# astrodeepnet/debvader

Measured on AMD Instinct MI355X. Metric: galaxy stamps/sec (train fwd+bwd+Adam) 59x59x6, higher is better.
Workload: dtype f32; 1 GPU; BASELINE configs[1]: 6-band 59x59 stamps, batch=256 per GPU, latent_dim=32, filters [32,64,128,256], fp32, stage-1 VAE train step; global_batch=256, per_gpu_batch=256, parallelism=dp1

## Files before the change

### debvader_amd/csrc/common.h

```cpp
#pragma once
#include <hip/hip_runtime.h>
#include <stdint.h>
#include <stddef.h>
#include <memory>
#include <utility>
#include <vector>

namespace dv {

enum : int {
  OK = 0,
  E_INVALID = -1,
  E_HIP = -2,
  E_NOMEM = -3,
  E_RCCL = -4,
  E_STATE = -5,
  E_NODEVICE = -6,
};

void set_error(const char* fmt, ...);
int hip_fail(hipError_t e, const char* what, const char* file, int line);

#define DV_HIP(call)                                                     \
  do {                                                                   \
// ... 65 lines not shown
__device__ __forceinline__ void dv_philox4x32_10(unsigned c0, unsigned c1, unsigned c2, unsigned c3, unsigned k0,
                                                 unsigned k1, unsigned out[4]) {
#pragma unroll
  for (int r = 0; r < 10; ++r) {
    unsigned long long p0 = 0xD2511F53ull * c0, p1 = 0xCD9E8D57ull * c2;
    unsigned n0 = (unsigned)(p1 >> 32) ^ c1 ^ k0, n1 = (unsigned)p1;
    unsigned n2 = (unsigned)(p0 >> 32) ^ c3 ^ k1, n3 = (unsigned)p0;
    c0 = n0; c1 = n1; c2 = n2; c3 = n3;
    k0 += 0x9E3779B9u;
    k1 += 0xBB67AE85u;
  }
  out[0] = c0; out[1] = c1; out[2] = c2; out[3] = c3;
}
__device__ __forceinline__ float dv_philox_normal(unsigned row, unsigned col, unsigned stream, unsigned long long seed) {
  unsigned r[4];
  dv_philox4x32_10(row, col >> 2, stream, 0u, (unsigned)seed, (unsigned)(seed >> 32), r);
  const int a = col & 3;
  const float u1 = ((float)r[a & ~1] + 1.0f) * 2.3283064365386963e-10f;
  const float u2 = ((float)r[(a & ~1) + 1] + 1.0f) * 2.3283064365386963e-10f;
  const float rad = sqrtf(-2.0f * logf(fminf(u1, 1.0f)));
  float sn, cs;
  sincosf(6.283185307179586f * u2, &sn, &cs);
  return (a & 1) ? rad * sn : rad * cs;
}
#endif

#define DV_MAX_TAPS 25
struct TapTab {
  int n;
  unsigned t[DV_MAX_TAPS];
};

struct GConvParams {
  const float* X;
  const float* W;
  float* U;
  float* A;
  const float* bias;
  const float* alpha;
  int NB, Hin, Win, Cin;
  int Hout, Wout, Cout;
  int Hc, Wc;
  int sin, sout, ph, pw;
  int ntaps;
  TapTab xt;
  int M, K;
// ... 227 lines not shown
struct DetectDevSrc {
  const double* fields_dev;
  int nb, band;
  const int32_t* which_h;
};
int scene_detect_dev(const DetectDevSrc& src, int M, int H, int W, double thresh, double cont, int minarea, int nthresh,
                     int back_size, int back_filter, const double* kernel_h, int kh, int kw, int64_t workspace_bytes,
                     int64_t cap, int64_t* n_out, int64_t* offsets_h, double* globalrms_h, int32_t* field_h,
                     int32_t* parent_h, int32_t* npix_h, double* peak_h, double* flux_h, double* x_h, double* y_h,
                     hipStream_t s);

struct GStripParams {
  const float* X;
  const float* W;
  float* U;
  float* A;
  const float* bias;
  const float* alpha;
  const float* zero;
  int NB, H, Wd, Cin, Cout;
  unsigned long long tapcode, wtcode;
  int epi;
  int R, patch_floats, strips_per_stamp, nstrips, strips_per_wg;
};
int launch_gconv_strip(GStripParams p, bool nmajor, hipStream_t s);
int launch_gconv_strip8(GStripParams p, hipStream_t s);

struct WinoParams {
  const float* X;
  const float* Ut;
  float* U;
  float* A;
  const float* bias;
  const float* alpha;
  const float* zero;
  int NB, H, Cin, Cout;
  int epi;
  int nbh, nct, NC, groups, items, items_per_wg;
};
struct WinoWDesc {
  const float* W;
  float* Ut;
  int Cin, Cout, nmajor;
  int wtmap[9];
};
struct WinoWgradParams {
  const float* X;
  const float* Y;
// ... 210 lines not shown
```

### debvader_amd/csrc/engine.hip

```cpp
#include <rccl/rccl.h>
#include <math.h>
#include <stdarg.h>
#include <stdio.h>
#include <stdlib.h>
#include <string.h>
#include <unistd.h>

#include <algorithm>
#include <string>
#include <thread>
#include <map>
#include <memory>
#include <mutex>
#include <optional>
#include <set>
#include <vector>
#ifdef DV_DEBUG_EXPORTS
#include <functional>
#endif

#include "../../include/debvader_hip.h"
#ifdef DV_DEBUG_EXPORTS
#include "../../include/debvader_hip_debug.h"
#endif
// ... 334 lines not shown
  hipEvent_t ev_red = nullptr;
  hipStream_t lane_stream[3] = {nullptr, nullptr, nullptr};
  hipEvent_t ev_lane[3] = {nullptr, nullptr, nullptr};
  hipEvent_t ev_ready = nullptr, ev_join = nullptr, ev_buf[3] = {nullptr, nullptr, nullptr};
  hipEvent_t ev_dec = nullptr, ev_enc = nullptr, ev_comm = nullptr, ev_small = nullptr, ev_small2 = nullptr;
  hipEvent_t ev_mid = nullptr;
  hipEvent_t ev_wred = nullptr;
  ncclComm_t comm = nullptr;
  bool cprof_on = false;
  std::vector<std::pair<hipEvent_t, hipEvent_t>> cprof_comm, cprof_wait;
  std::vector<hipEvent_t> cprof_pool;
  bool fake_peers = false;
  float* red_dev = nullptr;
  std::vector<dv_model*> models;
};

struct ProfRec {
  int klass;
  int fam;
  hipEvent_t a, b;
};
enum {
  PF_NONE = -1, PF_GCONV2 = 0, PF_GCONV_S2, PF_GSTRIP, PF_GSTRIP8, PF_GCONV, PF_WGRAD, PF_WSTRIP, PF_BCONV, PF_BWGRAD,
  PF_WINO, PF_WINOW, PF_BTRUNK, PF_COUNT
};
static const char* const kProfFamName[PF_COUNT] = {
    "gconv2_kernel", "gconv_s2_kernel", "gconv_strip_kernel", "gconv_strip8_kernel", "gconv_kernel", "wgrad_kernel",
    "wgrad_strip_kernel / wgrad_strip8_kernel", "bconv_kernel", "bwgrad_kernel", "wino_conv4_kernel / wino_conv_kernel", "wino_wgrad_kernel",
    "bgemm_kernel / bgemm_tn_kernel"};

struct DataSlot {
  float* x = nullptr;
  float* y = nullptr;
  int64_t n = 0;
  bool streamed = false;
  const char *hx = nullptr, *hy = nullptr;
  bool x64 = false, y64 = false;
  int64_t sx = 0, sy = 0;
  int64_t h2d_bytes = 0;
  hipEvent_t ready = nullptr;
};

struct StreamRing {
  static constexpr int kDepth = 4;
  static constexpr int kRel = 4;
  dv::DevBuf<float> dev[kDepth];
  dv::PinBuf<float> host[kDepth];
  size_t yoff = 0;
  hipStream_t copy = nullptr;
  hipEvent_t h2d[kDepth] = {};
  hipEvent_t rel[kDepth][kRel] = {};
  bool queued[kDepth] = {};
// ... 186 lines not shown
  int ws_last = -1;
  std::vector<float*> gbufs;
  float* gpool = nullptr;
  float* ws1x = nullptr;
  int ws_nreg = 3;
  size_t ws_region_cap = 0;
  int ws_count = 0;
  float* ws_head = nullptr;
  bool defer_loss_sums = false, loss_pending = false;
  int loss_blocks = 0, loss_NB = 0;
#ifdef DV_DEBUG_EXPORTS
  std::vector<std::function<int()>> exp_deferred;
#endif
  hipStream_t ws_last_rs = nullptr;
  bool step_pool_tried = false;
  size_t max_act_elems = 0;
  bool main_marked = false;
  unsigned long long* seed_dev = nullptr;
  bool use_seed_dev = false;
  bool infer_graph = false;
  uint64_t graph_epoch = ~(uint64_t)0;
  bool tiny_call = false;
  bool keep_outputs = false;
  std::map<int, hipGraphExec_t> infer_graphs;
  std::map<int, int> infer_seen;
  bool normalise = false;
  bool mse_sample = false;
  unsigned long long cur_seed = 0;
  bool early_adam = false;
  float lr_t_step = 0.f;
  size_t adam_done_from = 0;
  size_t enc_reduced_from = 0;
  float* zero_page = nullptr;
  int* idx_dev = nullptr;
  DataSlot slots[2];
  StreamRing* ring = nullptr;
  int lastB = 0;
  bool prof_on = false;
  std::vector<ProfRec> prof;
  std::vector<hipEvent_t> ev_pool;
  int64_t prof_n[3] = {0, 0, 0};
  int64_t prof_launches[3] = {0, 0, 0};
  bool prof_open = false;
  int prof_open_fam = -1;
  int64_t fam_launches[16] = {0};
  double fam_ms[16] = {0}, fam_flops[16] = {0}, fam_exec[16] = {0}, fam_bytes[16] = {0};
// ... 1089 lines not shown
  }
  const float* in = xn;
  for (int j = 0; j < 2 * A.L; ++j) {
    int hin, cin, hout, cout, st;
    A.enc_layer(j, &hin, &cin, &hout, &cout, &st);
    const int ksz = A.enc_ksz(j);
    int pb = same_pad_before(hin, ksz, st, nullptr);
    const float* W = j == 0 ? m->W1p : P + A.specs[A.enc_k(j)].off;
    int cin_phys = j == 0 ? A.C0p : cin;
    const size_t e_out = (size_t)hout * hout * cout;
    DV_TRY(gconv_fprop(m, in, W, false, P + A.specs[A.enc_b(j)].off, P + A.specs[A.enc_al(j)].off,
                       keep_u ? LANE(m->enc_u[j], e_out) : nullptr, LANE(m->enc_a[j], e_out), exp_epi(keep_u, hout), NB, hin,
                       cin_phys, hout, cout, st, pb, false, nullptr, nullptr, ksz));
    in = LANE(m->enc_a[j], e_out);
  }
  {
    ProfScope ps(m, 2);
    if (!exp_skip_small()) DV_TRY(launch_prelu_fwd(in, P + A.specs[A.enc_flat_al()].off, LANE(m->flat_a, A.flat), NB, A.flat, s));
  }
  return gconv_fprop(m, LANE(m->flat_a, A.flat), enc_dense_w(m), false, enc_dense_b(m),
                     nullptr, LANE(m->t, A.twp), nullptr, 1, NB, 1, A.flat, 1, A.twp, 1, 0, true);
}

static int decoder_forward(dv_model* m, int NB, bool keep_u) {
  if (m->bf.on) return bf_decoder_forward(m, NB, keep_u);
  const Arch& A = m->A;
  hipStream_t s = fwd_stream(m);
  float* P = m->P;
  {
    ProfScope ps(m, 2);
    if (!exp_skip_small() && !m->ain_done)
      DV_TRY(launch_prelu_fwd(LANE(m->z, A.dp), P + A.specs[A.D0].off, LANE(m->dec_ain, A.dp), NB, A.dp, s));
    m->ain_done = false;
  }
  DV_TRY(gconv_fprop(m, LANE(m->dec_ain, A.dp), dec_dense0_w(m), false, P + A.specs[A.D0 + 2].off,
                     P + A.specs[A.D0 + 3].off, keep_u ? LANE(m->dec_uh, A.dec_hidden) : nullptr,
                     LANE(m->dec_ah, A.dec_hidden), 2, NB, 1, A.dp, 1, A.dec_hidden, 1, 0, true));
  int r = A.w0 * A.w0 * A.cfg.filters[A.L - 1];
  DV_TRY(gconv_fprop(m, LANE(m->dec_ah, A.dec_hidden), P + A.specs[A.D0 + 4].off, false, P + A.specs[A.D0 + 5].off,
                     P + A.specs[A.D0 + 6].off, keep_u ? LANE(m->dec_ur, r) : nullptr, LANE(m->dec_ar, r), 2, NB, 1,
                     A.dec_hidden, 1, r, 1, 0, true));
  const float* in = LANE(m->dec_ar, r);
  for (int j = 0; j < 2 * A.L; ++j) {
    int hin, cin, hout, cout, st;
    A.dec_layer(j, &hin, &cin, &hout, &cout, &st);
    const int ksz = A.dec_ksz(j);
    int pb = same_pad_before(hout, ksz, st, nullptr);
    const size_t e_out = (size_t)hout * hout * cout;
    DV_TRY(gconv_dgrad(m, in, P + A.specs[A.dec_k(j)].off, true, P + A.specs[A.dec_b(j)].off,
                       P + A.specs[A.dec_al(j)].off, keep_u ? LANE(m->dec_u[j], e_out) : nullptr,
                       LANE(m->dec_a[j], e_out), exp_epi(keep_u, hout), NB, hin, cin, hout, cout, st, pb, nullptr, nullptr, ksz));
    in = LANE(m->dec_a[j], e_out);
  }
  return gconv_fprop(m, in, m->Whp, false, m->bhp, nullptr, LANE(m->tpre, (size_t)A.dec_out * A.dec_out * A.C2p),
                     nullptr, 1, NB, A.dec_out, A.cfg.filters[0], A.dec_out, A.C2p, 1, 1);
}

static int sampler_forward(dv_model* m, int NB, bool gen, uint64_t seed, unsigned stream_id, unsigned row0,
                           bool want_std, int rep_nb = 0) {
  const Arch& A = m->A;
  SamplerParams sp;
  memset(&sp, 0, sizeof sp);
  sp.t = LANE(m->t, A.twp);
  sp.eps = LANE(m->eps, A.dp);
  sp.z = LANE(m->z, A.dp);
  sp.ldt = A.twp;
  sp.ldz = A.dp;
  sp.kl = LANE(m->kl, 1);
  sp.stddev = want_std ? LANE(m->zstd, A.dp) : nullptr;
  sp.NB = NB;
  sp.d = A.d;
  sp.diag_shift = A.cfg.diag_shift;
  sp.gen = gen ? 1 : 0;
  sp.seed = seed;
  sp.stream = stream_id;
  sp.row0 = row0 + (unsigned)m->b0;
  sp.rep_nb = rep_nb;
  sp.seed_ptr = m->use_seed_dev ? m->seed_dev : nullptr;
// ... 23 lines not shown
  hp.idx = idx ? idx + m->b0 : nullptr;
  hp.first = first + m->b0;
  hp.dt = want_grad ? LANE(m->gA, head_e) : nullptr;
  hp.loc = want_out ? LANE(m->loc, stamp) : nullptr;
  hp.scale = want_out ? LANE(m->scale, stamp) : nullptr;
  hp.part = m->ws3 + (size_t)part_block0 * 2;
  hp.NB = NB;
  hp.Hd = A.dec_out;
  hp.H = A.H;
  hp.nb = A.C;
  hp.crop0 = A.crop0;
  hp.ld = A.C2p;
  hp.sigma_floor = A.cfg.sigma_floor;
  hp.gscale = (float)(1.0 / ((double)Bg * A.H * A.H * A.C));
  hp.mse_sample = m->mse_sample ? 1 : 0;
  hp.mse_row0 = m->b0;
  hp.mse_stream = DV_MSE_STREAM + (unsigned)m->ctx->rank;
  hp.mse_seed = m->cur_seed;
}

static int head_lane(dv_model* m, const float* ysrc, const int* idx, int first, int NB, int Bg, bool want_grad,
                     bool want_out, int part_block0, int* nblk) {
  if (m->bf.on) return bf_head_lane(m, ysrc, idx, first, NB, Bg, want_grad, want_out, part_block0, nblk);
  HeadParams hp;
  head_params(m, hp, ysrc, idx, first, NB, Bg, want_grad, want_out, part_block0);
  ProfScope ps(m, 2);
  return launch_head(hp, fwd_stream(m), nblk);
}

static int forward_all(dv_model* m, const float* xsrc, const float* ysrc, const int* idx, int first, int NB, int Bg,
                       bool training, bool upd_moving, bool keep_u, const float* eps_host, uint64_t seed,
                       unsigned stream_id, unsigned row0, bool want_std, bool want_grad, bool want_out,
                       bool run_encoder = true) {
  const Arch& A = m->A;
  dv_ctx* cx = m->ctx;
  hipStream_t s = cx->stream;
  m->cur_seed = seed;
  if (!m->bf.on) DV_TRY(wino_refresh_all(m, s));
#ifdef DV_DEBUG_EXPORTS
  if (!m->exp_deferred.empty()) {
    if (ysrc && want_grad && cx->aux_stream) {
      m->wstream = cx->aux_stream;
      m->main_marked = false;
      for (auto& f : m->exp_deferred) DV_TRY(f());
      if (m->bf.on) DV_TRY(bf_flush_wred(m, nullptr));
      m->wstream = s;
    }
    m->exp_deferred.clear();
  }
// ... 22 lines not shown
        set_error("batch %d needs %d forward lanes of <= %ld stamps; at most %d are available (DV_FWD_LANES)", NB, nlanes,
                  cap, cx->lane_stream[1] ? 4 : (cx->lane_stream[0] ? 3 : 2));
        return E_INVALID;
      }
    }
  }
  const int per = nlanes > 1 ? ((NB / nlanes + 31) / 32) * 32 : NB;
  int blk_done = 0, st = OK;
  hipStream_t lstream[4] = {nullptr, cx->aux_stream, cx->lane_stream[0], cx->lane_stream[1]};
  if (nlanes > 1) {
    DV_HIP(hipEventRecord(cx->ev_ready, s));
    for (int lane = 1; lane < nlanes; ++lane) DV_HIP(hipStreamWaitEvent(lstream[lane], cx->ev_ready, 0));
  }
  for (int lane = 0; lane < nlanes && st == OK; ++lane) {
    m->b0 = lane * per;
    m->lane_id = lane;
    m->cs = lstream[lane];
    const int nb = std::min(per, NB - m->b0);
    if (nb <= 0) break;
    int nblk = 0;
    if (run_encoder) st = encoder_forward(m, xsrc, idx, first, nb, keep_u, true);
    if (st == OK && run_encoder) st = sampler_forward(m, nb, eps_host == nullptr, seed, stream_id, row0, want_std);
    if (st == OK && m->bf.on) bf_head_fuse_request(m, ysrc, idx, first, nb, Bg, want_grad, want_out, blk_done);
    if (st == OK) st = decoder_forward(m, nb, keep_u);
    if (st == OK) st = head_lane(m, ysrc, idx, first, nb, Bg, want_grad, want_out, blk_done, &nblk);
    blk_done += nblk;
    if (st == OK && lane > 0) {
      if (hipEventRecord(cx->ev_lane[lane - 1], lstream[lane]) != hipSuccess ||
          hipStreamWaitEvent(s, cx->ev_lane[lane - 1], 0) != hipSuccess)
        st = E_HIP;
    }
  }
  m->b0 = 0;
  m->lane_id = 0;
  m->cs = nullptr;
  if (st != OK) return st;
  const int blk0 = blk_done, blk1 = 0;
  if (ysrc && m->defer_loss_sums) {
    m->loss_blocks = blk0 + blk1;
    m->loss_NB = NB;
    m->loss_pending = true;
  } else if (ysrc && !(exp_skip_tail() & 2)) {
    ProfScope ps(m, 2, s);
    DV_TRY(launch_reduce_rows_f64(m->ws3, blk0 + blk1, 2, m->scal, 1.0f, s));
    DV_TRY(launch_reduce_rows_f64(m->kl, NB, 1, m->scal + 2, 1.0f, s));
  }
// ... 1786 lines not shown
  ALLOC(m->loc, Bc * A.H * A.H * A.C + 4);
  ALLOC(m->scale, Bc * A.H * A.H * A.C + 4);
  ALLOC(m->gA, Bc * max_act);
  ALLOC(m->gB, Bc * max_act);
  ALLOC(m->gC, Bc * max_act);
  {
    float* sd = nullptr;
    ALLOC(sd, 4);
    m->seed_dev = reinterpret_cast<unsigned long long*>(sd);
  }
  m->gbufs = {m->gA, m->gB, m->gC};
  m->max_act_elems = Bc * max_act;
  size_t max_w = 0;
  for (auto& s : A.specs)
    if (s.ndim >= 2) max_w = std::max(max_w, s.count);
  max_w = std::max(max_w, k0sq * A.C0p * cfg->filters[0]);
  m->ws1_elems = std::max((size_t)32 << 20, (max_w + 1024) * 3);
  ALLOC(m->ws1, m->ws1_elems);
  m->ws4_elems = (size_t)4 * 16 * Bc * std::max((size_t)A.flat, (size_t)A.tw);
  ALLOC(m->ws4, m->ws4_elems);
  m->wstream = ctx->stream;
  if (getenv("DV_NO_OVERLAP")) m->overlap_wgrad = false;
  if (getenv("DV_NO_FWD_SPLIT")) m->split_forward = false;
  if (g_fuse_prelu_bwd) m->no_fuse = false;
  m->arena_elems = 0;
  for (auto& sp : A.specs)
    if (sp.name.size() > 6 && sp.name.compare(sp.name.size() - 6, 6, "/alpha") == 0)
      m->arena_elems += (size_t)std::max<size_t>(33, bf16 ? 2 * ((Bc + 63) / 64) + 2 : 0) * ((sp.count + 3) & ~(size_t)3) + 65536;
  ALLOC(m->arena, m->arena_elems);
  m->ws2_elems = std::max((size_t)1 << 20, max_act * 16);
  ALLOC(m->ws2, m->ws2_elems);
  size_t head_blocks = (Bc * A.dec_out * A.dec_out + 255) / 256;
  m->ws3_elems = std::max((size_t)1 << 20, head_blocks * 2 + 64);
  m->ws3_elems = std::max(m->ws3_elems, (size_t)64 * std::max((size_t)A.flat, r));
  m->ws3_elems = std::max(m->ws3_elems, (std::max<size_t>((Bc + 2047) / 2048, 64) + 1) * A.twp);
  m->ws3_elems = std::max(m->ws3_elems, ((Bc * (size_t)A.H * A.H + 1023) / 1024 + 1) * (2 * DV_BN_MAXC));
  ALLOC(m->ws3, m->ws3_elems);
  if (bf16) ALLOC(m->ws_head, m->ws3_elems);
  ALLOC(m->scal, 16);
  ALLOC(m->zero_page, 64);
  ALLOC(m->bnstate, 4 * DV_BN_MAXC);
  ALLOC(m->bnsums, 2 * DV_BN_MAXC);
  ALLOC(m->bn_pre_sums, 2 * DV_BN_MAXC);
  m->bn_pre_part_elems = (size_t)(2 * DV_BN_MAXC) * (((size_t)Bc * A.H * A.H + 1023) / 1024 + 16);
  ALLOC(m->bn_pre_part, m->bn_pre_part_elems);
  for (int k = 0; k < 3; ++k)
// ... 424 lines not shown
    auto run_forward = [&]() -> int {
      if (m->normalise) DV_TRY(launch_normalise(m->stage_x, (long)nb * stamp, false, s));
      DV_TRY(forward_all(m, m->stage_x, nullptr, nullptr, 0, nb, nb, false, false, false, eps ? eps + o * A.d : nullptr,
                         seed, (unsigned)m->ctx->rank, (unsigned)o, zstd != nullptr, false, true));
      if (m->normalise && loc) DV_TRY(launch_normalise(m->loc, (long)nb * stamp, true, s));
      return OK;
    };
    const bool graphable = m->infer_graph && nb < 64 && N <= m->Bc && !eps && m->seed_dev != nullptr;
    if (graphable && m->graph_epoch != m->param_epoch) {
      for (auto& kv : m->infer_graphs) (void)hipGraphExecDestroy(kv.second);
      m->infer_graphs.clear();
      m->infer_seen.clear();
      m->graph_epoch = m->param_epoch;
    }
    if (graphable) {
      const int key = nb | (zstd ? 1 << 20 : 0) | (m->normalise ? 1 << 21 : 0) | (loc ? 1 << 22 : 0);
      m->use_seed_dev = true;
      const unsigned long long seed_host = seed;
      int st = OK;
      if (hipMemcpyAsync(m->seed_dev, &seed_host, sizeof seed_host, hipMemcpyHostToDevice, s) != hipSuccess) st = E_HIP;
      auto it = m->infer_graphs.find(key);
      if (st == OK && it != m->infer_graphs.end()) {
        if (hipGraphLaunch(it->second, s) != hipSuccess) st = E_HIP;
      } else if (st == OK && m->infer_seen[key]++ >= 1) {
        hipGraph_t g = nullptr;
        hipGraphExec_t ge = nullptr;
        if (hipStreamBeginCapture(s, hipStreamCaptureModeRelaxed) != hipSuccess) st = E_HIP;
        if (st == OK) {
          st = run_forward();
          const hipError_t ce = hipStreamEndCapture(s, &g);
          if (st == OK && ce != hipSuccess) st = E_HIP;
        }
        if (st == OK && hipGraphInstantiate(&ge, g, nullptr, nullptr, 0) != hipSuccess) st = E_HIP;
        if (g) (void)hipGraphDestroy(g);
        if (st == OK) {
          m->infer_graphs[key] = ge;
          if (hipGraphLaunch(ge, s) != hipSuccess) st = E_HIP;
        }
      } else if (st == OK) {
        st = run_forward();
      }
      m->use_seed_dev = false;
      if (st != OK) {
        if (st == E_HIP) set_error("graph-captured inference forward failed: %s", hipGetErrorString(hipGetLastError()));
        return st;
      }
// ... 1489 lines not shown
  else if (n == "scale") { src = m->scale; elems = B * A.H * A.H * A.C; }
  else if (n == "head_pre") {
    elems = B * A.dec_out * A.dec_out * 2 * A.C;
    if (nbytes != elems * sizeof(float)) {
      set_error("activation head_pre holds %zu bytes, caller passed %zu", elems * sizeof(float), nbytes);
      return DV_E_INVALID;
    }
    DV_HIP(hipSetDevice(m->ctx->device));
    DV_HIP(hipStreamSynchronize(m->ctx->stream));
    if (m->bf.on && m->bf.tpre_stale) {
      set_error("head_pre is not stored by a step that runs the head in the head conv's epilogue: keep the outputs "
                "(dv_model_set_keep_outputs) or set DV_BF_HEAD_FUSED=0");
      return DV_E_STATE;
    }
    if (m->bf.on) {
      const size_t Pn = (size_t)A.dec_out * A.dec_out, NBp = (size_t)m->bf.NBp, HC = (size_t)A.C2p;
      std::vector<float> tmp(Pn * NBp * HC);
      DV_HIP(hipMemcpy(tmp.data(), m->bf.tpre32, tmp.size() * sizeof(float), hipMemcpyDeviceToHost));
      for (size_t b = 0; b < B; ++b)
        for (size_t px = 0; px < Pn; ++px)
          memcpy(host + (b * Pn + px) * 2 * A.C, tmp.data() + (px * NBp + b) * HC, 2 * A.C * sizeof(float));
      return DV_OK;
    }
    DV_HIP(hipMemcpy2D(host, 2 * A.C * sizeof(float), m->tpre, A.C2p * sizeof(float), 2 * A.C * sizeof(float),
                       B * A.dec_out * A.dec_out, hipMemcpyDeviceToHost));
    return DV_OK;
  }
  else if (m->bf.on) {
    const void* bsrc = nullptr;
    size_t Pn = 0, Cn = 0;
    if (n == "xn") { bsrc = m->bf.xh; Pn = (size_t)A.H * A.H; Cn = 16; }
    else if (n == "dec_in") { bsrc = m->bf.dec_in; Pn = (size_t)A.w0 * A.w0; Cn = A.cfg.filters[A.L - 1]; }
    else if (n == "d_dec_in") { bsrc = m->bf.d_dec_in; Pn = (size_t)A.w0 * A.w0; Cn = A.cfg.filters[A.L - 1]; }
    else if (n == "dec_ur") {
      if (!m->bf.trunk_mfma) {
        set_error("activation dec_ur: the dense trunk of this configuration runs on the fp32 kernels");
        return DV_E_STATE;
      }
      bsrc = m->bf.dec_ur; Pn = (size_t)A.w0 * A.w0; Cn = A.cfg.filters[A.L - 1];
    }
    else if (n == "d_head_pre") { bsrc = m->bf.dt; Pn = (size_t)A.dec_out * A.dec_out; Cn = (size_t)A.C2p; }
    else if (n.size() > 6 && (n.rfind("enc_du", 0) == 0 || n.rfind("dec_du", 0) == 0)) {
      const int j = atoi(n.c_str() + 6);
      if (j < 0 || j >= 2 * A.L || (int)m->bf.du_enc.size() != 2 * A.L) return DV_E_INVALID;
      int hin, cin, hout, cout, s;
      if (n[0] == 'e') A.enc_layer(j, &hin, &cin, &hout, &cout, &s); else A.dec_layer(j, &hin, &cin, &hout, &cout, &s);
// ... 501 lines not shown
```

### debvader_amd/csrc/gconv_strip.hip

```cpp
#include "common.h"
#include <stdlib.h>

namespace dv {

typedef const __attribute__((address_space(1))) void* gs_gptr_t;
typedef __attribute__((address_space(3))) void* gs_lptr_t;

namespace {
constexpr int GS_WAVES = 8;
constexpr int GS_THREADS = 64 * GS_WAVES;
constexpr int GS_MAXG = 8;
constexpr int GS_LDC = 36;
__device__ __forceinline__ int gs_dh(unsigned long long code, int t) { return (int)((code >> (4 * t)) & 3) - 1; }
__device__ __forceinline__ int gs_dw(unsigned long long code, int t) { return (int)((code >> (4 * t + 2)) & 3) - 1; }
__device__ __forceinline__ int gs_wt(unsigned long long code, int t) { return (int)((code >> (4 * t)) & 15); }
}

template <int CIN, int COUT, bool NMAJOR>
__global__ __launch_bounds__(GS_THREADS, 1) void gconv_strip_kernel(const GStripParams p) {
  constexpr int CQ = CIN / 4;
  constexpr int QG = CIN / 16;
  constexpr int NSTEPS = 9 * QG;
  constexpr int SWS = CQ == 8 ? 1 : 2;
#define GS_SW(idx) (((idx) >> SWS) & (CQ - 1))
  constexpr int TN = COUT / 16;
  extern __shared__ __attribute__((aligned(16))) float smem[];
  float* patch = smem;
  float* wts = smem + 2 * p.patch_floats;
  float* stage = wts + 9 * COUT * CIN;

  const int tid = threadIdx.x, lane = tid & 63;
  const int wave = __builtin_amdgcn_readfirstlane(tid >> 6);
  const int l15 = lane & 15, lg = lane >> 4;
  const int W = p.Wd, PW = W + 2;
  const int strip_px = p.R * W;

  for (int e = tid; e < 9 * COUT * CQ; e += GS_THREADS) {
    const int t = e / (COUT * CQ), rem = e - t * (COUT * CQ);
    const int wt = gs_wt(p.wtcode, t);
    if (NMAJOR) {
      const int n = rem / CQ, kq = rem - n * CQ;
      f32x4 v = {0.f, 0.f, 0.f, 0.f};
// ... 59 lines not shown
  const int s_begin = blockIdx.x * p.strips_per_wg;
  const int s_end = min(p.nstrips, s_begin + p.strips_per_wg);
  if (s_begin < s_end) issue_dma(s_begin, 0);
  int buf = 0;
  float* stg = stage + wave * (16 * GS_LDC);
  constexpr int F4 = COUT / 4;
  constexpr int ROWS_IT = 64 / F4;
  constexpr int NIT = 16 / ROWS_IT;
  const int ef4 = lane % F4, ecol = ef4 * 4;
  f32x4 bias4 = {0.f, 0.f, 0.f, 0.f};
  if (p.epi >= 1 && ecol < p.Cout) bias4 = *reinterpret_cast<const f32x4*>(p.bias + ecol);
  f32x4 alr[2][NIT];
  auto prefetch_alpha = [&](int i0) {
#pragma unroll
    for (int mb = 0; mb < 2; ++mb)
#pragma unroll
      for (int it = 0; it < NIT; ++it) {
        const int px = wave * 32 + mb * 16 + lane / F4 + it * ROWS_IT;
        const int pr = px / W, pc = px - pr * W;
        const bool ok = px < strip_px && i0 + pr < p.H && ecol < p.Cout;
        alr[mb][it] = *reinterpret_cast<const f32x4*>(p.alpha + (ok ? (unsigned)(((i0 + pr) * W + pc) * p.Cout + ecol) : 0u));
      }
  };
  auto epi_half = [&](const f32x4 (&ac)[2][TN], int mb, int n, int i0) {
#pragma unroll
    for (int tn = 0; tn < TN; ++tn)
#pragma unroll
      for (int r = 0; r < 4; ++r) stg[(lg * 4 + r) * GS_LDC + tn * 16 + l15] = ac[mb][tn][r];
    __builtin_amdgcn_s_waitcnt(0xC07F);
    __builtin_amdgcn_wave_barrier();
    const int col = ecol;
#pragma unroll
    for (int it = 0; it < NIT; ++it) {
      const int rr = lane / F4 + it * ROWS_IT;
      const int px = wave * 32 + mb * 16 + rr;
      const int pr = px / W, pc = px - pr * W;
      if (px >= strip_px || i0 + pr >= p.H || col >= p.Cout) continue;
      const unsigned aoff = (unsigned)(((i0 + pr) * W + pc) * p.Cout + col);
      const unsigned ooff = (unsigned)(n * p.H * W * p.Cout) + aoff;
      f32x4 v = *reinterpret_cast<const f32x4*>(stg + rr * GS_LDC + col);
      v += bias4;
      if (p.U) *reinterpret_cast<f32x4*>(p.U + ooff) = v;
      if (p.epi == 2) {
        const f32x4 al = alr[mb][it];
        f32x4 o;
#pragma unroll
        for (int k = 0; k < 4; ++k) o[k] = v[k] > 0.f ? v[k] : al[k] * v[k];
        *reinterpret_cast<f32x4*>(p.A + ooff) = o;
      }
    }
    __builtin_amdgcn_wave_barrier();
  };
  f32x4 pacc[2][TN];
  int pn = 0, pi0 = 0;
  bool have_prev = false;
  for (int sidx = s_begin; sidx < s_end; ++sidx) {
    __builtin_amdgcn_s_waitcnt(0x0F70);
    __syncthreads();
    if (sidx + 1 < s_end) issue_dma(sidx + 1, buf ^ 1);
    if (have_prev && p.epi == 2) prefetch_alpha(pi0);
    const float* P = patch + buf * p.patch_floats;

    f32x4 acc[2][TN];
#pragma unroll
    for (int a = 0; a < 2; ++a)
#pragma unroll
      for (int b = 0; b < TN; ++b) acc[a][b] = (f32x4){0.f, 0.f, 0.f, 0.f};

    auto load_frags = [&](int step, f32x4 (&af)[2], f32x4 (&bf)[TN]) {
      const int t = step / QG, qg = step - t * QG;
      const int shift = gs_dh(p.tapcode, t) * PW + gs_dw(p.tapcode, t);
#pragma unroll
      for (int mb = 0; mb < 2; ++mb) {
        const int L = L0[mb] + shift;
        af[mb] = *reinterpret_cast<const f32x4*>(P + L * CIN + (((qg * 4 + lg) ^ GS_SW(L)) << 2));
      }
#pragma unroll
      for (int tn = 0; tn < TN; ++tn)
        bf[tn] = *reinterpret_cast<const f32x4*>(wts + t * COUT * CIN + nbase[tn] + (((qg * 4 + lg) ^ nsw[tn]) << 2));
    };
    auto mfma_step = [&](const f32x4 (&af)[2], const f32x4 (&bf)[TN]) {
#pragma unroll
      for (int jj = 0; jj < 4; ++jj)
#pragma unroll
        for (int mb = 0; mb < 2; ++mb)
#pragma unroll
          for (int tn = 0; tn < TN; ++tn)
            acc[mb][tn] = __builtin_amdgcn_mfma_f32_16x16x4f32(af[mb][jj], bf[tn][jj], acc[mb][tn], 0, 0, 0);
    };
    f32x4 a0[2], b0[TN], a1[2], b1[TN];
    constexpr int H1 = (NSTEPS / 4) & ~1, H2 = H1 + ((NSTEPS / 3) & ~1);
    load_frags(0, a0, b0);
#pragma unroll
    for (int step = 0; step < NSTEPS; step += 2) {
      if (step + 1 < NSTEPS) load_frags(step + 1, a1, b1);
      mfma_step(a0, b0);
      if (step + 2 < NSTEPS) load_frags(step + 2, a0, b0);
      if (step + 1 < NSTEPS) mfma_step(a1, b1);
      if (step == H1 && have_prev) epi_half(pacc, 0, pn, pi0);
      if (step == H2 && have_prev) epi_half(pacc, 1, pn, pi0);
    }
#pragma unroll
    for (int a = 0; a < 2; ++a)
#pragma unroll
      for (int b2 = 0; b2 < TN; ++b2) pacc[a][b2] = acc[a][b2];
    pn = sidx / p.strips_per_stamp;
    pi0 = (sidx - pn * p.strips_per_stamp) * p.R;
    have_prev = true;
    buf ^= 1;
  }
  if (have_prev) {
    if (p.epi == 2) prefetch_alpha(pi0);
    epi_half(pacc, 0, pn, pi0);
    epi_half(pacc, 1, pn, pi0);
  }
}

#undef GS_SW

__global__ __launch_bounds__(GS_THREADS, 4) void gconv_strip8_kernel(const GStripParams p) {
  constexpr int CIN = 8, COUT = 32, TN = 2, NST = 5;
  extern __shared__ __attribute__((aligned(16))) float smem[];
  float* patch = smem;
  float* wts = smem + 2 * p.patch_floats;
  float* stage = wts + NST * COUT * 16;
  const int tid = threadIdx.x, lane = tid & 63;
  const int wave = __builtin_amdgcn_readfirstlane(tid >> 6);
  const int l15 = lane & 15, lg = lane >> 4;
  const int W = p.Wd, PW = W + 2;
  const int strip_px = p.R * W;

  for (int e = tid; e < NST * COUT * 16; e += GS_THREADS) {
    const int st = e / (COUT * 16), rem = e - st * (COUT * 16);
    const int n = rem >> 4, k16 = rem & 15;
    const int t = 2 * st + (k16 >> 3), c = k16 & 7;
    const float v = t < 9 ? p.W[(t * CIN + c) * COUT + n] : 0.f;
    wts[(st * COUT + n) * 16 + ((((k16 >> 2) ^ ((n >> 2) & 3)) << 2) | (k16 & 3))] = v;
// ... 164 lines not shown
  if (R > p.H) R = p.H;
  const int PW = p.Wd + 2;
  const int slots = (R + 2) * PW * 2;
  if ((slots + 63) / 64 > 2 * GS_WAVES) return 1;
  p.R = R;
  p.patch_floats = ((slots + 63) / 64) * 256;
  p.strips_per_stamp = (p.H + R - 1) / R;
  p.nstrips = p.NB * p.strips_per_stamp;
  const int target = 512;
  p.strips_per_wg = (p.nstrips + target - 1) / target;
  const int grid = (p.nstrips + p.strips_per_wg - 1) / p.strips_per_wg;
  const size_t smem = ((size_t)2 * p.patch_floats + (size_t)5 * 32 * 16 + (size_t)GS_WAVES * 16 * GS_LDC) * sizeof(float);
  static bool attr_set = false;
  if (!attr_set) {
    DV_HIP(hipFuncSetAttribute(reinterpret_cast<const void*>(gconv_strip8_kernel),
                               hipFuncAttributeMaxDynamicSharedMemorySize, (int)smem));
    attr_set = true;
  }
  hipLaunchKernelGGL(gconv_strip8_kernel, dim3(grid), dim3(GS_THREADS), smem, s, p);
  DV_HIP(hipGetLastError());
  return OK;
}

template <int CIN, int COUT, bool NMAJOR>
static int launch_gs(const GStripParams& p, int grid, size_t smem, hipStream_t s) {
  static bool attr_set = false;
  auto kern = gconv_strip_kernel<CIN, COUT, NMAJOR>;
  if (!attr_set) {
    DV_HIP(hipFuncSetAttribute(reinterpret_cast<const void*>(kern), hipFuncAttributeMaxDynamicSharedMemorySize,
                               (int)smem));
    attr_set = true;
  }
  hipLaunchKernelGGL(kern, dim3(grid), dim3(GS_THREADS), smem, s, p);
  DV_HIP(hipGetLastError());
  return OK;
}

int launch_gconv_strip(GStripParams p, bool nmajor, hipStream_t s) {
  if ((p.Cin != 32 && p.Cin != 16) || (p.Cout != 32 && p.Cout != 16) || !p.zero) return 1;
  if (p.Cin == 16 && p.Cout != 32) return 1;
  if (p.Wd < 8 || p.Wd > 64 || p.H < 1 || p.epi < 0 || p.epi > 2) return 1;
  if ((long)p.NB * p.H * p.Wd * 32 >= (1L << 30)) return 1;
  const int cout_pad = p.Cout <= 16 ? 16 : 32;
  int R = 256 / p.Wd;
  if (R > p.H) R = p.H;
  if (R < 1) return 1;
  const int PW = p.Wd + 2;
  const int slots = (R + 2) * PW * (p.Cin / 4);
  if ((slots + 63) / 64 > GS_MAXG * GS_WAVES) return 1;
  p.R = R;
  p.patch_floats = ((slots + 63) / 64) * 256;
  p.strips_per_stamp = (p.H + R - 1) / R;
  p.nstrips = p.NB * p.strips_per_stamp;
  static int cus = 0;
  if (!cus) {
    int dev = 0;
    hipDeviceProp_t prop;
    if (hipGetDevice(&dev) != hipSuccess || hipGetDeviceProperties(&prop, dev) != hipSuccess) return 1;
    cus = prop.multiProcessorCount > 0 ? prop.multiProcessorCount : 256;
  }
  p.strips_per_wg = (p.nstrips + cus - 1) / cus;
  const int grid = (p.nstrips + p.strips_per_wg - 1) / p.strips_per_wg;
  const size_t smem = ((size_t)2 * p.patch_floats + (size_t)9 * cout_pad * p.Cin + (size_t)GS_WAVES * 16 * GS_LDC) * sizeof(float);
  if (smem > 160 * 1024) return 1;
  if (p.Cin == 16) return nmajor ? launch_gs<16, 32, true>(p, grid, smem, s) : launch_gs<16, 32, false>(p, grid, smem, s);
  if (cout_pad == 16) return nmajor ? launch_gs<32, 16, true>(p, grid, smem, s) : launch_gs<32, 16, false>(p, grid, smem, s);
  return nmajor ? launch_gs<32, 32, true>(p, grid, smem, s) : launch_gs<32, 32, false>(p, grid, smem, s);
}

}
```

### debvader_amd/csrc/pointwise.hip

```cpp
#include <algorithm>

#include "common.h"

namespace dv {

__device__ __forceinline__ float wave_sum(float v) {
#pragma unroll
  for (int o = 32; o > 0; o >>= 1) v += __shfl_down(v, o, 64);
  return v;
}

__device__ __forceinline__ float block_sum(float v, float* sh ) {
  v = wave_sum(v);
  __syncthreads();
  if ((threadIdx.x & 63) == 0) sh[threadIdx.x >> 6] = v;
  __syncthreads();
  return sh[0] + sh[1] + sh[2] + sh[3];
}

__global__ __launch_bounds__(256) void reduce_rows_f64_kernel(const float* __restrict__ part, int nrows, int ld,
                                                              float* __restrict__ out, float scale) {
  __shared__ double sh[256];
  const int c = blockIdx.x;
  double acc = 0.0;
// ... 447 lines not shown
    const f32x4 z4 = {0.f, 0.f, 0.f, 0.f};
    if (dtp && p.ld == 16) dtp[3] = z4;
    if (!in) {
      if (dtp) {
        dtp[0] = z4;
        dtp[1] = z4;
        dtp[2] = z4;
      }
    } else {
      const f32x4* tp = reinterpret_cast<const f32x4*>(p.tpre + pp * p.ld);
      const f32x4 t0 = tp[0], t1 = tp[1], t2 = tp[2];
      const float t[12] = {t0[0], t0[1], t0[2], t0[3], t1[0], t1[1], t1[2], t1[3], t2[0], t2[1], t2[2], t2[3]};
      const long opix = ((long)b * p.H + h) * p.H + w;
      float yv[6] = {0.f, 0.f, 0.f, 0.f, 0.f, 0.f};
      if (p.y) {
        long row = p.idx ? p.idx[b] : p.first + b;
        const f32x2* yp = reinterpret_cast<const f32x2*>(p.y + ((row * p.H + h) * p.H + w) * 6);
        const f32x2 y0 = yp[0], y1 = yp[1], y2 = yp[2];
        yv[0] = y0[0]; yv[1] = y0[1]; yv[2] = y1[0]; yv[3] = y1[1]; yv[4] = y2[0]; yv[5] = y2[1];
      }
      float loc[6], sig[6], d[12];
#pragma unroll
      for (int c = 0; c < 6; ++c) {
        loc[c] = fmaxf(t[c], 0.f);
        sig[c] = p.sigma_floor + fmaxf(t[6 + c], 0.f);
        d[c] = d[6 + c] = 0.f;
        if (p.y) {
          const float inv = 1.0f / sig[c];
          const float df = yv[c] - loc[c];
          const float r = df * inv;
          nll += 0.5f * r * r + logf(sig[c]) + 0.91893853320467274178f;
          if (p.mse_sample) {
            const float dsm = df - sig[c] * dv_philox_normal((unsigned)(p.mse_row0 + b), (unsigned)((h * p.H + w) * 6 + c), p.mse_stream, p.mse_seed);
            se += dsm * dsm;
          } else {
            se += df * df;
          }
          d[c] = t[c] > 0.f ? -(r * inv) * p.gscale : 0.f;
          d[6 + c] = t[6 + c] > 0.f ? (inv - r * r * inv) * p.gscale : 0.f;
        }
      }
      if (dtp) {
        dtp[0] = (f32x4){d[0], d[1], d[2], d[3]};
        dtp[1] = (f32x4){d[4], d[5], d[6], d[7]};
        dtp[2] = (f32x4){d[8], d[9], d[10], d[11]};
      }
      if (p.loc) {
        f32x2* lp = reinterpret_cast<f32x2*>(p.loc + opix * 6);
        lp[0] = (f32x2){loc[0], loc[1]};
        lp[1] = (f32x2){loc[2], loc[3]};
        lp[2] = (f32x2){loc[4], loc[5]};
      }
      if (p.scale) {
        f32x2* sp = reinterpret_cast<f32x2*>(p.scale + opix * 6);
        sp[0] = (f32x2){sig[0], sig[1]};
        sp[1] = (f32x2){sig[2], sig[3]};
        sp[2] = (f32x2){sig[4], sig[5]};
      }
    }
  }
  float a = block_sum(nll, sh);
  float b2 = block_sum(se, sh);
  if (threadIdx.x == 0 && p.part) {
// ... 576 lines not shown
```

Before: 55660 stamps/s.

## Fuse Gaussian-likelihood head into final decoder strip convolution epilogue

Adds a HEAD variant of the strip convolution kernel that computes the loss head (NLL, MSE partials and gradients w.r.t. pre-activation) directly in the epilogue from staged accumulators. Labels are prefetched during the MMA loop, and the head kernel launch plus the tpre write and readback are skipped during training. Because tpre is no longer written, a lazy restore path recomputes it when outputs are read on the host. This adds template complexity and staleness-tracking state.

```diff
diff --git a/debvader_amd/csrc/common.h b/debvader_amd/csrc/common.h
--- a/debvader_amd/csrc/common.h
+++ b/debvader_amd/csrc/common.h
@@ -111,6 +111,32 @@
   float sn, cs;
   sincosf(6.283185307179586f * u2, &sn, &cs);
   return (a & 1) ? rad * sn : rad * cs;
+}
+struct HeadBand {
+  float loc, sig, dl, ds;
+};
+__device__ __forceinline__ HeadBand dv_head_band(float tl, float ts, float yv, bool has_y, float sigma_floor, float gscale,
+                                                 int mse_sample, unsigned mse_row, unsigned mse_elem, unsigned mse_stream,
+                                                 unsigned long long mse_seed, float& nll, float& se) {
+  HeadBand o;
+  o.loc = fmaxf(tl, 0.f);
+  o.sig = sigma_floor + fmaxf(ts, 0.f);
+  o.dl = o.ds = 0.f;
+  if (has_y) {
+    const float inv = 1.0f / o.sig;
+    const float df = yv - o.loc;
+    const float r = df * inv;
+    nll += 0.5f * r * r + logf(o.sig) + 0.91893853320467274178f;
+    if (mse_sample) {
+      const float dsm = df - o.sig * dv_philox_normal(mse_row, mse_elem, mse_stream, mse_seed);
+      se += dsm * dsm;
+    } else {
+      se += df * df;
+    }
+    o.dl = tl > 0.f ? -(r * inv) * gscale : 0.f;
+    o.ds = ts > 0.f ? (inv - r * r * inv) * gscale : 0.f;
+  }
+  return o;
 }
 #endif
 
@@ -384,8 +410,16 @@
   unsigned long long tapcode, wtcode;
   int epi;
   int R, patch_floats, strips_per_stamp, nstrips, strips_per_wg;
-};
-int launch_gconv_strip(GStripParams p, bool nmajor, hipStream_t s);
+  int head;
+  const float* hy;
+  const int* hidx;
+  int hfirst;
+  float* hdt;
+  float* hpart;
+  int hH, hcrop0;
+  float hsigma_floor, hgscale;
+};
+int launch_gconv_strip(GStripParams p, bool nmajor, hipStream_t s, int* head_rows = nullptr);
 int launch_gconv_strip8(GStripParams p, hipStream_t s);
 
 struct WinoParams {
diff --git a/debvader_amd/csrc/engine.hip b/debvader_amd/csrc/engine.hip
--- a/debvader_amd/csrc/engine.hip
+++ b/debvader_amd/csrc/engine.hip
@@ -380,12 +380,12 @@
 };
 enum {
   PF_NONE = -1, PF_GCONV2 = 0, PF_GCONV_S2, PF_GSTRIP, PF_GSTRIP8, PF_GCONV, PF_WGRAD, PF_WSTRIP, PF_BCONV, PF_BWGRAD,
-  PF_WINO, PF_WINOW, PF_BTRUNK, PF_COUNT
+  PF_WINO, PF_WINOW, PF_BTRUNK, PF_HEAD, PF_COUNT
 };
 static const char* const kProfFamName[PF_COUNT] = {
     "gconv2_kernel", "gconv_s2_kernel", "gconv_strip_kernel", "gconv_strip8_kernel", "gconv_kernel", "wgrad_kernel",
     "wgrad_strip_kernel / wgrad_strip8_kernel", "bconv_kernel", "bwgrad_kernel", "wino_conv4_kernel / wino_conv_kernel", "wino_wgrad_kernel",
-    "bgemm_kernel / bgemm_tn_kernel"};
+    "bgemm_kernel / bgemm_tn_kernel", "head6_kernel / head_kernel"};
 
 struct DataSlot {
   float* x = nullptr;
@@ -618,6 +618,16 @@
   uint64_t graph_epoch = ~(uint64_t)0;
   bool tiny_call = false;
   bool keep_outputs = false;
+  bool head_fused = true;
+  struct {
+    bool req = false;
+    const float* ysrc = nullptr;
+    const int* idx = nullptr;
+    int first = 0, Bg = 0, part_block0 = 0;
+    bool want_grad = false, want_out = false;
+  } hfuse;
+  int hfuse_rows = 0;
+  int tpre_stale_nb = 0;
   std::map<int, hipGraphExec_t> infer_graphs;
   std::map<int, int> infer_seen;
   bool normalise = false;
@@ -1753,6 +1763,56 @@
                      nullptr, LANE(m->t, A.twp), nullptr, 1, NB, 1, A.flat, 1, A.twp, 1, 0, true);
 }
 
+static void head_params(dv_model* m, HeadParams& hp, const float* ysrc, const int* idx, int first, int NB, int Bg,
+                        bool want_grad, bool want_out, int part_block0);
+static void head_fuse_request(dv_model* m, const float* ysrc, const int* idx, int first, int Bg, bool want_grad,
+                              bool want_out, int part_block0) {
+  const Arch& A = m->A;
+  m->hfuse.req = false;
+  if (!m->head_fused || m->bf.on || A.C != 6 || A.C2p != 16 || A.cfg.filters[0] != 32 || A.dec_out < 8 || A.dec_out > 64 ||
+      g_no_special || g_force_v1 || !m->no_fuse || !m->zero_page || exp_skip_tail())
+    return;
+  if (!ysrc || !want_grad || want_out || m->mse_sample) return;
+  m->hfuse.req = true;
+  m->hfuse.ysrc = ysrc;
+  m->hfuse.idx = idx;
+  m->hfuse.first = first;
+  m->hfuse.Bg = Bg;
+  m->hfuse.want_grad = want_grad;
+  m->hfuse.want_out = want_out;
+  m->hfuse.part_block0 = part_block0;
+}
+
+static int head_conv_fused(dv_model* m, const float* in, int NB) {
+  const Arch& A = m->A;
+  HeadParams hp;
+  head_params(m, hp, m->hfuse.ysrc, m->hfuse.idx, m->hfuse.first, NB, m->hfuse.Bg, m->hfuse.want_grad, m->hfuse.want_out,
+              m->hfuse.part_block0);
+  const Taps tp = taps_fprop(1, 3);
+  if (tp.n != 9) return 1;
+  GStripParams g;
+  memset(&g, 0, sizeof g);
+  g.X = in; g.W = m->Whp; g.bias = m->bhp; g.zero = m->zero_page;
+  g.NB = NB; g.H = A.dec_out; g.Wd = A.dec_out; g.Cin = A.cfg.filters[0]; g.Cout = A.C2p;
+  g.tapcode = tp.tapcode; g.wtcode = tp.wtcode; g.epi = 1;
+  g.head = 1;
+  g.hy = hp.y; g.hidx = hp.idx; g.hfirst = hp.first; g.hdt = hp.dt; g.hpart = hp.part;
+  g.hH = hp.H; g.hcrop0 = hp.crop0; g.hsigma_floor = hp.sigma_floor; g.hgscale = hp.gscale;
+  const long max_rows = (long)NB * A.dec_out;
+  if ((size_t)(m->hfuse.part_block0 + max_rows) * 2 > m->ws3_elems) return 1;
+  const double flops = 2.0 * NB * A.dec_out * A.dec_out * 9 * (double)A.cfg.filters[0] * (double)(2 * A.C);
+  int rows = 0, r;
+  {
+    ProfScope ps(m, 0, nullptr, PF_GSTRIP, flops);
+    r = launch_gconv_strip(g, false, fwd_stream(m), &rows);
+    if (r > 0) prof_uncount(m, 0, PF_GSTRIP, flops);
+  }
+  if (r != 0) return r;
+  m->hfuse_rows = rows;
+  m->tpre_stale_nb = std::max(m->b0 == 0 ? 0 : m->tpre_stale_nb, m->b0 + NB);
+  return OK;
+}
+
 static int decoder_forward(dv_model* m, int NB, bool keep_u) {
   if (m->bf.on) return bf_decoder_forward(m, NB, keep_u);
   const Arch& A = m->A;
@@ -1783,8 +1843,33 @@
                        LANE(m->dec_a[j], e_out), exp_epi(keep_u, hout), NB, hin, cin, hout, cout, st, pb, nullptr, nullptr, ksz));
     in = LANE(m->dec_a[j], e_out);
   }
+  m->hfuse_rows = 0;
+  if (m->hfuse.req) {
+    m->hfuse.req = false;
+    const int r = head_conv_fused(m, in, NB);
+    if (r <= 0) return r;
+  }
+  if (m->b0 == 0) m->tpre_stale_nb = 0;
   return gconv_fprop(m, in, m->Whp, false, m->bhp, nullptr, LANE(m->tpre, (size_t)A.dec_out * A.dec_out * A.C2p),
                      nullptr, 1, NB, A.dec_out, A.cfg.filters[0], A.dec_out, A.C2p, 1, 1);
+}
+
+static int tpre_restore(dv_model* m) {
+  const Arch& A = m->A;
+  if (m->bf.on || m->tpre_stale_nb <= 0) return OK;
+  const size_t in_e = (size_t)A.dec_out * A.dec_out * A.cfg.filters[0];
+  const int cap = (int)std::max<size_t>(1, ((((size_t)1 << 30) - 1) / in_e) & ~(size_t)31);
+  const int total = m->tpre_stale_nb;
+  int st = OK;
+  for (int b = 0; b < total && st == OK; b += cap) {
+    m->b0 = b;
+    st = gconv_fprop(m, LANE(m->dec_a[2 * A.L - 1], in_e), m->Whp, false, m->bhp, nullptr,
+                     LANE(m->tpre, (size_t)A.dec_out * A.dec_out * A.C2p), nullptr, 1, std::min(cap, total - b), A.dec_out,
+                     A.cfg.filters[0], A.dec_out, A.C2p, 1, 1);
+  }
+  m->b0 = 0;
+  if (st == OK) m->tpre_stale_nb = 0;
+  return st;
 }
 
 static int sampler_forward(dv_model* m, int NB, bool gen, uint64_t seed, unsigned stream_id, unsigned row0,
@@ -1854,9 +1939,14 @@
 static int head_lane(dv_model* m, const float* ysrc, const int* idx, int first, int NB, int Bg, bool want_grad,
                      bool want_out, int part_block0, int* nblk) {
   if (m->bf.on) return bf_head_lane(m, ysrc, idx, first, NB, Bg, want_grad, want_out, part_block0, nblk);
+  if (m->hfuse_rows > 0) {
+    if (nblk) *nblk = m->hfuse_rows;
+    m->hfuse_rows = 0;
+    return OK;
+  }
   HeadParams hp;
   head_params(m, hp, ysrc, idx, first, NB, Bg, want_grad, want_out, part_block0);
-  ProfScope ps(m, 2);
+  ProfScope ps(m, 2, nullptr, PF_HEAD);
   return launch_head(hp, fwd_stream(m), nblk);
 }
 
@@ -1925,6 +2015,7 @@
     if (run_encoder) st = encoder_forward(m, xsrc, idx, first, nb, keep_u, true);
     if (st == OK && run_encoder) st = sampler_forward(m, nb, eps_host == nullptr, seed, stream_id, row0, want_std);
     if (st == OK && m->bf.on) bf_head_fuse_request(m, ysrc, idx, first, nb, Bg, want_grad, want_out, blk_done);
+    if (st == OK && !m->bf.on) head_fuse_request(m, ysrc, idx, first, Bg, want_grad, want_out, blk_done);
     if (st == OK) st = decoder_forward(m, nb, keep_u);
     if (st == OK) st = head_lane(m, ysrc, idx, first, nb, Bg, want_grad, want_out, blk_done, &nblk);
     blk_done += nblk;
@@ -3757,6 +3848,7 @@
   m->wstream = ctx->stream;
   if (getenv("DV_NO_OVERLAP")) m->overlap_wgrad = false;
   if (getenv("DV_NO_FWD_SPLIT")) m->split_forward = false;
+  if (const char* hf = getenv("DV_HEAD_FUSED")) m->head_fused = atoi(hf) != 0;
   if (g_fuse_prelu_bwd) m->no_fuse = false;
   m->arena_elems = 0;
   for (auto& sp : A.specs)
@@ -4227,6 +4319,7 @@
       auto it = m->infer_graphs.find(key);
       if (st == OK && it != m->infer_graphs.end()) {
         if (hipGraphLaunch(it->second, s) != hipSuccess) st = E_HIP;
+        m->tpre_stale_nb = 0;
       } else if (st == OK && m->infer_seen[key]++ >= 1) {
         hipGraph_t g = nullptr;
         hipGraphExec_t ge = nullptr;
@@ -5762,6 +5855,10 @@
           memcpy(host + (b * Pn + px) * 2 * A.C, tmp.data() + (px * NBp + b) * HC, 2 * A.C * sizeof(float));
       return DV_OK;
     }
+    if (m->tpre_stale_nb > 0) {
+      DV_TRY(tpre_restore(m));
+      DV_HIP(hipStreamSynchronize(m->ctx->stream));
+    }
     DV_HIP(hipMemcpy2D(host, 2 * A.C * sizeof(float), m->tpre, A.C2p * sizeof(float), 2 * A.C * sizeof(float),
                        B * A.dec_out * A.dec_out, hipMemcpyDeviceToHost));
     return DV_OK;
diff --git a/debvader_amd/csrc/gconv_strip.hip b/debvader_amd/csrc/gconv_strip.hip
--- a/debvader_amd/csrc/gconv_strip.hip
+++ b/debvader_amd/csrc/gconv_strip.hip
@@ -5,6 +5,8 @@
 
 typedef const __attribute__((address_space(1))) void* gs_gptr_t;
 typedef __attribute__((address_space(3))) void* gs_lptr_t;
+typedef const __attribute__((address_space(4))) int* gs_cptr_t;
+typedef float f32x2 __attribute__((ext_vector_type(2)));
 
 namespace {
 constexpr int GS_WAVES = 8;
@@ -16,8 +18,9 @@
 __device__ __forceinline__ int gs_wt(unsigned long long code, int t) { return (int)((code >> (4 * t)) & 15); }
 }
 
-template <int CIN, int COUT, bool NMAJOR>
+template <int CIN, int COUT, bool NMAJOR, bool HEAD>
 __global__ __launch_bounds__(GS_THREADS, 1) void gconv_strip_kernel(const GStripParams p) {
+  static_assert(!HEAD || (COUT == 16 && !NMAJOR), "the head epilogue is the 16-column k-major form");
   constexpr int CQ = CIN / 4;
   constexpr int QG = CIN / 16;
   constexpr int NSTEPS = 9 * QG;
@@ -123,6 +126,29 @@
         alr[mb][it] = *reinterpret_cast<const f32x4*>(p.alpha + (ok ? (unsigned)(((i0 + pr) * W + pc) * p.Cout + ecol) : 0u));
       }
   };
+  const int hq = lane & 3, hrr = lane >> 2;
+  float hbias[4] = {0.f, 0.f, 0.f, 0.f};
+  f32x2 ylab[2] = {{0.f, 0.f}, {0.f, 0.f}};
+  f32x2 ylabn[2] = {{0.f, 0.f}, {0.f, 0.f}};
+  float h_nll = 0.f, h_se = 0.f;
+  if (HEAD && hq < 3) {
+    hbias[0] = p.bias[2 * hq];
+    hbias[1] = p.bias[2 * hq + 1];
+    hbias[2] = p.bias[6 + 2 * hq];
+    hbias[3] = p.bias[7 + 2 * hq];
+  }
+  auto prefetch_labels = [&](int n, int i0) {
+    const long row = p.hidx ? (long)((gs_cptr_t)p.hidx)[n] : (long)p.hfirst + n;
+#pragma unroll
+    for (int mb = 0; mb < 2; ++mb) {
+      const int px = wave * 32 + mb * 16 + hrr;
+      const int pr = px / W, pc = px - pr * W;
+      const int h = i0 + pr - p.hcrop0, w = pc - p.hcrop0;
+      const bool ok = hq < 3 && px < strip_px && (unsigned)h < (unsigned)p.hH && (unsigned)w < (unsigned)p.hH;
+      const float* src = ok ? p.hy + (((row * p.hH + h) * p.hH + w) * 6 + 2 * hq) : p.zero;
+      asm volatile("global_load_dwordx2 %0, %1, off" : "=v"(ylabn[mb]) : "v"(src) : "memory");
+    }
+  };
   auto epi_half = [&](const f32x4 (&ac)[2][TN], int mb, int n, int i0) {
 #pragma unroll
     for (int tn = 0; tn < TN; ++tn)
@@ -131,6 +157,39 @@
     __builtin_amdgcn_s_waitcnt(0xC07F);
     __builtin_amdgcn_wave_barrier();
     const int col = ecol;
+    if constexpr (HEAD) {
+      const int px = wave * 32 + mb * 16 + hrr;
+      const int pr = px / W, pc = px - pr * W;
+      const bool live = px < strip_px && i0 + pr < p.H;
+      const int h = i0 + pr - p.hcrop0, w = pc - p.hcrop0;
+      float* row = stg + hrr * GS_LDC;
+      if (hq < 3) {
+        f32x2 dl = {0.f, 0.f}, ds = {0.f, 0.f};
+        if (live && (unsigned)h < (unsigned)p.hH && (unsigned)w < (unsigned)p.hH) {
+          f32x2 tl = *reinterpret_cast<const f32x2*>(row + 2 * hq);
+          f32x2 ts = *reinterpret_cast<const f32x2*>(row + 6 + 2 * hq);
+          tl[0] += hbias[0]; tl[1] += hbias[1]; ts[0] += hbias[2]; ts[1] += hbias[3];
+#pragma unroll
+          for (int k = 0; k < 2; ++k) {
+            const HeadBand o = dv_head_band(tl[k], ts[k], ylab[mb][k], true, p.hsigma_floor, p.hgscale, 0, 0u, 0u, 0u, 0ull,
+                                            h_nll, h_se);
+            dl[k] = o.dl; ds[k] = o.ds;
+          }
+        }
+        *reinterpret_cast<f32x2*>(row + 2 * hq) = dl;
+        *reinterpret_cast<f32x2*>(row + 6 + 2 * hq) = ds;
+      } else {
+        *reinterpret_cast<f32x4*>(row + 12) = (f32x4){0.f, 0.f, 0.f, 0.f};
+      }
+      __builtin_amdgcn_s_waitcnt(0xC07F);
+      __builtin_amdgcn_wave_barrier();
+      if (live) {
+        const unsigned ooff = (unsigned)(n * p.H * W * 16) + (unsigned)(((i0 + pr) * W + pc) * 16 + col);
+        *reinterpret_cast<f32x4*>(p.hdt + ooff) = *reinterpret_cast<const f32x4*>(row + col);
+      }
+      __builtin_amdgcn_wave_barrier();
+      return;
+    }
 #pragma unroll
     for (int it = 0; it < NIT; ++it) {
       const int rr = lane / F4 + it * ROWS_IT;
@@ -160,6 +219,10 @@
     __syncthreads();
     if (sidx + 1 < s_end) issue_dma(sidx + 1, buf ^ 1);
     if (have_prev && p.epi == 2) prefetch_alpha(pi0);
+    if (HEAD) {
+      const int cn = sidx / p.strips_per_stamp;
+      prefetch_labels(cn, (sidx - cn * p.strips_per_stamp) * p.R);
+    }
     const float* P = patch + buf * p.patch_floats;
 
     f32x4 acc[2][TN];
@@ -201,6 +264,12 @@
       if (step == H1 && have_prev) epi_half(pacc, 0, pn, pi0);
       if (step == H2 && have_prev) epi_half(pacc, 1, pn, pi0);
     }
+    if (HEAD) {
+      __builtin_amdgcn_s_waitcnt(0x0F70);
+      asm volatile("" : "+v"(ylabn[0]), "+v"(ylabn[1]));
+      ylab[0] = ylabn[0];
+      ylab[1] = ylabn[1];
+    }
 #pragma unroll
     for (int a = 0; a < 2; ++a)
 #pragma unroll
@@ -214,6 +283,25 @@
     if (p.epi == 2) prefetch_alpha(pi0);
     epi_half(pacc, 0, pn, pi0);
     epi_half(pacc, 1, pn, pi0);
+  }
+  if constexpr (HEAD) {
+#pragma unroll
+    for (int o = 32; o >= 1; o >>= 1) {
+      h_nll += __shfl_xor(h_nll, o, 64);
+      h_se += __shfl_xor(h_se, o, 64);
+    }
+    __syncthreads();
+    if (lane == 0) {
+      stage[2 * wave] = h_nll;
+      stage[2 * wave + 1] = h_se;
+    }
+    __syncthreads();
+    if (tid < 2) {
+      float tot = 0.f;
+#pragma unroll
+      for (int k = 0; k < GS_WAVES; ++k) tot += stage[2 * k + tid];
+      p.hpart[blockIdx.x * 2 + tid] = tot;
+    }
   }
 }
 
@@ -424,10 +512,10 @@
   return OK;
 }
 
-template <int CIN, int COUT, bool NMAJOR>
+template <int CIN, int COUT, bool NMAJOR, bool HEAD = false>
 static int launch_gs(const GStripParams& p, int grid, size_t smem, hipStream_t s) {
   static bool attr_set = false;
-  auto kern = gconv_strip_kernel<CIN, COUT, NMAJOR>;
+  auto kern = gconv_strip_kernel<CIN, COUT, NMAJOR, HEAD>;
   if (!attr_set) {
     DV_HIP(hipFuncSetAttribute(reinterpret_cast<const void*>(kern), hipFuncAttributeMaxDynamicSharedMemorySize,
                                (int)smem));
@@ -438,8 +526,12 @@
   return OK;
 }
 
-int launch_gconv_strip(GStripParams p, bool nmajor, hipStream_t s) {
+int launch_gconv_strip(GStripParams p, bool nmajor, hipStream_t s, int* head_rows) {
   if ((p.Cin != 32 && p.Cin != 16) || (p.Cout != 32 && p.Cout != 16) || !p.zero) return 1;
+  if (p.head) {
+    if (p.Cin != 32 || p.Cout != 16 || nmajor || p.epi != 1 || !p.bias || !p.hpart || !p.hy || !p.hdt || p.H != p.Wd) return 1;
+    if (p.hH < 1 || p.hcrop0 < 0 || p.hcrop0 + p.hH > p.H) return 1;
+  }
   if (p.Cin == 16 && p.Cout != 32) return 1;
   if (p.Wd < 8 || p.Wd > 64 || p.H < 1 || p.epi < 0 || p.epi > 2) return 1;
   if ((long)p.NB * p.H * p.Wd * 32 >= (1L << 30)) return 1;
@@ -466,6 +558,10 @@
   const size_t smem = ((size_t)2 * p.patch_floats + (size_t)9 * cout_pad * p.Cin + (size_t)GS_WAVES * 16 * GS_LDC) * sizeof(float);
   if (smem > 160 * 1024) return 1;
   if (p.Cin == 16) return nmajor ? launch_gs<16, 32, true>(p, grid, smem, s) : launch_gs<16, 32, false>(p, grid, smem, s);
+  if (p.head) {
+    if (head_rows) *head_rows = grid;
+    return launch_gs<32, 16, false, true>(p, grid, smem, s);
+  }
   if (cout_pad == 16) return nmajor ? launch_gs<32, 16, true>(p, grid, smem, s) : launch_gs<32, 16, false>(p, grid, smem, s);
   return nmajor ? launch_gs<32, 32, true>(p, grid, smem, s) : launch_gs<32, 32, false>(p, grid, smem, s);
 }
diff --git a/debvader_amd/csrc/pointwise.hip b/debvader_amd/csrc/pointwise.hip
--- a/debvader_amd/csrc/pointwise.hip
+++ b/debvader_amd/csrc/pointwise.hip
@@ -493,23 +493,13 @@
       float loc[6], sig[6], d[12];
 #pragma unroll
       for (int c = 0; c < 6; ++c) {
-        loc[c] = fmaxf(t[c], 0.f);
-        sig[c] = p.sigma_floor + fmaxf(t[6 + c], 0.f);
-        d[c] = d[6 + c] = 0.f;
-        if (p.y) {
-          const float inv = 1.0f / sig[c];
-          const float df = yv[c] - loc[c];
-          const float r = df * inv;
-          nll += 0.5f * r * r + logf(sig[c]) + 0.91893853320467274178f;
-          if (p.mse_sample) {
-            const float dsm = df - sig[c] * dv_philox_normal((unsigned)(p.mse_row0 + b), (unsigned)((h * p.H + w) * 6 + c), p.mse_stream, p.mse_seed);
-            se += dsm * dsm;
-          } else {
-            se += df * df;
-          }
-          d[c] = t[c] > 0.f ? -(r * inv) * p.gscale : 0.f;
-          d[6 + c] = t[6 + c] > 0.f ? (inv - r * r * inv) * p.gscale : 0.f;
-        }
+        const HeadBand o = dv_head_band(t[c], t[6 + c], yv[c], p.y != nullptr, p.sigma_floor, p.gscale, p.mse_sample,
+                                        (unsigned)(p.mse_row0 + b), (unsigned)((h * p.H + w) * 6 + c), p.mse_stream,
+                                        p.mse_seed, nll, se);
+        loc[c] = o.loc;
+        sig[c] = o.sig;
+        d[c] = o.dl;
+        d[6 + c] = o.ds;
       }
       if (dtp) {
         dtp[0] = (f32x4){d[0], d[1], d[2], d[3]};
```

New measurement: 56040 stamps/s, median of 6. Within noise of the previous version (+0.7%).
